# adamgreig/labrador-ldpc

Measured on AMD Instinct MI355X. Metric: decoded codewords/sec @25 min-sum iters, TM8192, Eb/N0=2dB; 1/2/4/8 GPU, higher is better.
Workload: dtype f32; 1 GPU; TM8192 f32 LLRs, 4194304 frames on 1 GPU = BASELINE config 4 whole, resident in HBM, max_iters 25 with early termination, AWGN Eb/N0 2.0 dB, 256 random codewords; code=TM8192, total_frames=4194304, frames_per_gpu=4194304, max_iters=25, parallelism=1 contiguous shard(s) of one batch, one process per GPU, no collective, kernel_variant=0, library_build=d4d007dc8df32436

## Files before the change

labrador_ldpc_amd/csrc/decode_ms_ops.hpp:

```cpp
#pragma once

#include <hip/hip_runtime.h>
#include <cfloat>
#include <cstdint>
#include <type_traits>

#include "decode_ms_util.hpp"

namespace ldpc {

template <class T> struct Ops;

template <> struct Ops<float> {
    using R = float;
    using E = float;
    LDPC_DEV static R zero() { return 0.0f; }
    LDPC_DEV static R maxval() { return FLT_MAX; }
    LDPC_DEV static R load(float x) { return __builtin_fminf(x + 0.0f, __builtin_inff()); }
    LDPC_DEV static R canon_late(R x) { return __builtin_fminf(x + 0.0f, __builtin_inff()); }
    LDPC_DEV static R keep_raw(float x) { return x; }
    LDPC_DEV static R load_nonan(float x) { return x + 0.0f; }
    LDPC_DEV static float store(R x) { return x; }
    LDPC_DEV static R from_lds(float x) { return x; }
    LDPC_DEV static int bits(R x) { return __float_as_int(x); }
    static constexpr bool SIGN_WORD_IS_BIT31_ONLY = true;
    LDPC_DEV static int sign_word(R x) { return __float_as_int(x) & (int)0x80000000; }
    LDPC_DEV static R add(R a, R b) { return a + b; }
    LDPC_DEV static R sub(R a, R b) { return a - b; }
    LDPC_DEV static R sub_nv(R a, R b) { return a - b; }
    LDPC_DEV static R mag(R x) { return __builtin_fabsf(x); }
    template <bool AX, bool AY>
    LDPC_DEV static R min2(R x, R y)
    {
        R d;
        if constexpr (AX && AY) asm("v_min_f32_e64 %0, |%1|, |%2|" : "=v"(d) : "v"(x), "v"(y));
        else if constexpr (AX) asm("v_min_f32_e64 %0, |%1|, %2" : "=v"(d) : "v"(x), "v"(y));
        else if constexpr (AY) asm("v_min_f32_e64 %0, %1, |%2|" : "=v"(d) : "v"(x), "v"(y));
        else asm("v_min_f32_e32 %0, %1, %2" : "=v"(d) : "v"(x), "v"(y));
        return d;
    }
    template <bool AX>
    LDPC_DEV static R min2_cap(R x)
    {
        R d;
        const float cap = FLT_MAX;
        if constexpr (AX) asm("v_min_f32_e64 %0, |%1|, %2" : "=v"(d) : "v"(x), "s"(cap));
        else asm("v_min_f32_e32 %0, %2, %1" : "=v"(d) : "v"(x), "s"(cap));
        return d;
    }
    template <bool AX, bool AY>
    LDPC_DEV static R min3_cap(R x, R y)
    {
        R d;
        const float cap = FLT_MAX;
        if constexpr (AX && AY) asm("v_min3_f32 %0, |%1|, |%2|, %3" : "=v"(d) : "v"(x), "v"(y), "s"(cap));
        else if constexpr (!AX && !AY) asm("v_min3_f32 %0, %1, %2, %3" : "=v"(d) : "v"(x), "v"(y), "s"(cap));
        else d = min2_cap<false>(min2<AX, AY>(x, y));
        return d;
    }
    template <bool AX, bool AY, bool AZ>
    LDPC_DEV static R min3(R x, R y, R z)
    {
        R d;
        if constexpr (AX && AY && AZ) asm("v_min3_f32 %0, |%1|, |%2|, |%3|" : "=v"(d) : "v"(x), "v"(y), "v"(z));
        else if constexpr (AX && AY) asm("v_min3_f32 %0, |%1|, |%2|, %3" : "=v"(d) : "v"(x), "v"(y), "v"(z));
        else if constexpr (!AX && !AY && !AZ) asm("v_min3_f32 %0, %1, %2, %3" : "=v"(d) : "v"(x), "v"(y), "v"(z));
        else d = min2<false, AZ>(min2<AX, AY>(x, y), z);
        return d;
    }
    LDPC_DEV static R with_sign(R m, int s)
    {
        return __int_as_float((__float_as_int(m) & 0x7FFFFFFF) | (s & (int)0x80000000));
    }
    LDPC_DEV static R select_zero(bool z, R x) { return z ? 0.0f : x; }
    LDPC_DEV static R keep_unless_negative(R p, R x)
    {
        R r;
        asm("v_subrev_co_u32_e32 %0, vcc, %2, %1\n\ts_nop 1\n\tv_cndmask_b32_e32 %0, 0, %3, vcc"
            : "=&v"(r) : "v"(p), "s"(0x80000001u), "v"(x) : "vcc");
        return r;
    }
    LDPC_DEV static bool drop(R nv, R old)
    {
        const int t = __builtin_amdgcn_bitop3_b32(__float_as_int(old), __float_as_int(nv), (int)0x80000000, 0x78);
        return __int_as_float(t) < 0.0f;
    }
    template <int FORM>
    LDPC_DEV static R clamp_to_side(R nv, R old, float big)
    {
        static_assert(FORM == 2 || FORM == 3, "clamp forms of the self-correction: 2, 3 (6: integer messages only, IntOps)");
        R x, r;
        if constexpr (FORM == 2) {
            asm("v_fma_f32 %0, %1, %2, %3" : "=v"(x) : "s"(big), "v"(old), "v"(nv));
        } else {
            asm("v_mul_legacy_f32_e64 %0, %1, %2" : "=v"(x) : "v"(old), "s"(__builtin_inff()));
            x = x + nv;
        }
        asm("v_med3_f32 %0, %1, 0, %2" : "=v"(r) : "v"(nv), "v"(x));
        return r;
    }
    template <int FORM>
    LDPC_DEV static R self_correct(R nv, R old)
    {
        if constexpr (FORM == 1) {
            const int t = __builtin_amdgcn_bitop3_b32(__float_as_int(old), __float_as_int(nv), (int)0x80000000, 0x78);
            return keep_unless_negative(__int_as_float(t), nv);
        } else {
            return select_zero(drop(nv, old), nv);
        }
    }
    template <bool BOUNDED, int FORM = 0>
    LDPC_DEV static R self_correct_b(R nv, R old)
    {
        if constexpr (BOUNDED && FORM >= 2) {
            return clamp_to_side<FORM>(nv, old, 0x1p126f);
        } else if constexpr (BOUNDED) {
            float p;
            asm("v_mul_f32_e32 %0, %1, %2" : "=v"(p) : "v"(nv), "v"(old));
            if constexpr (FORM == 1) return keep_unless_negative(p, nv);
            else return select_zero(p < 0.0f, nv);
        } else {
            return self_correct<(FORM == 1 ? 1 : 0)>(nv, old);
        }
    }
    LDPC_DEV static R apply_sign(R m, int s_all, int s_own)
    {
        return __int_as_float(__builtin_amdgcn_bitop3_b32(__float_as_int(m), s_all, s_own, 0x96));
    }
};

template <> struct Ops<double> {
    using R = double;
    using E = double;
    LDPC_DEV static R zero() { return 0.0; }
    LDPC_DEV static R maxval() { return DBL_MAX; }
    LDPC_DEV static R load(double x) { return __builtin_fmin(x + 0.0, __builtin_inf()); }
    LDPC_DEV static R canon_late(R x) { return __builtin_fmin(x + 0.0, __builtin_inf()); }
    LDPC_DEV static R keep_raw(double x) { return x; }
    LDPC_DEV static R load_nonan(double x) { return x + 0.0; }
    LDPC_DEV static double store(R x) { return x; }
    LDPC_DEV static R from_lds(double x) { return x; }
    LDPC_DEV static int bits(R x) { return __double2hiint(x); }
    static constexpr bool SIGN_WORD_IS_BIT31_ONLY = true;
    LDPC_DEV static int sign_word(R x) { return __double2hiint(x) & (int)0x80000000; }
    LDPC_DEV static R add(R a, R b) { return a + b; }
    LDPC_DEV static R sub(R a, R b) { return a - b; }
    LDPC_DEV static R sub_nv(R a, R b) { return a - b; }
    LDPC_DEV static R mag(R x) { return __builtin_fabs(x); }
    template <bool AX, bool AY>
    LDPC_DEV static R min2(R x, R y)
    {
        const R a = AX ? __builtin_fabs(x) : x, b = AY ? __builtin_fabs(y) : y;
        return __builtin_fmin(a, b);
    }
    template <bool AX> LDPC_DEV static R min2_cap(R x) { return min2<AX, false>(x, DBL_MAX); }
    template <bool AX, bool AY> LDPC_DEV static R min3_cap(R x, R y) { return min2<false, false>(min2<AX, AY>(x, y), DBL_MAX); }
    template <bool AX, bool AY, bool AZ>
    LDPC_DEV static R min3(R x, R y, R z) { return min2<false, AZ>(min2<AX, AY>(x, y), z); }
    template <int FORM>
    LDPC_DEV static R self_correct(R nv, R old)
    {
        return (old != 0.0 && (nv < 0.0) != (old < 0.0)) ? 0.0 : nv;
    }
    template <bool BOUNDED, int FORM = 0> LDPC_DEV static R self_correct_b(R nv, R old) { return self_correct<0>(nv, old); }
    LDPC_DEV static R apply_sign(R m, int s_all, int s_own)
    {
        return __hiloint2double(__double2hiint(m) ^ s_all ^ s_own, __double2loint(m));
    }
};

template <class I, int LO, int HI> struct IntOps : Ops<float> {
    LDPC_DEV static R maxval() { return (float)HI; }
    LDPC_DEV static R load(I x) { return (float)(int)x; }
    LDPC_DEV static R canon_late(R x) { return x; }
    LDPC_DEV static R keep_raw(I x) { return (float)(int)x; }
    LDPC_DEV static R load_nonan(I x) { return (float)(int)x; }
    LDPC_DEV static R clamp(R x) { return __builtin_amdgcn_fmed3f(x, (float)LO, (float)HI); }
    LDPC_DEV static R add(R a, R b) { return clamp(a + b); }
    LDPC_DEV static R sub(R a, R b) { return clamp(a - b); }
    LDPC_DEV static R sub_nv(R a, R b) { return a - b; }
    LDPC_DEV static R mag(R x) { return __builtin_fminf(__builtin_fabsf(x), (float)HI); }
    LDPC_DEV static bool drop(R nv, R old)
    {
        float p;
        asm("v_mul_f32_e32 %0, %1, %2" : "=v"(p) : "v"(nv), "v"(old));
        return p < 0.0f;
    }
    template <int FORM>
    LDPC_DEV static R self_correct(R nv, R old)
    {
        if constexpr (FORM == 6) {
            float sel, r;
            asm("v_fma_f32 %0, %1, %2, 1.0 clamp" : "=v"(sel) : "v"(nv), "v"(old));
            asm("v_fma_f32 %0, %1, %2, 0" : "=v"(r) : "v"(nv), "v"(sel));
            return r;
        } else if constexpr (FORM >= 2) {
            return Ops<float>::clamp_to_side<FORM>(nv, old, 0x1p20f);
        } else if constexpr (FORM == 1) {
            float p;
            asm("v_mul_f32_e32 %0, %1, %2" : "=v"(p) : "v"(nv), "v"(old));
            return Ops<float>::keep_unless_negative(p, nv);
        } else {
            return Ops<float>::select_zero(drop(nv, old), nv);
        }
    }
    template <bool BOUNDED, int FORM = 0> LDPC_DEV static R self_correct_b(R nv, R old) { return self_correct<FORM>(nv, old); }
    template <bool AX>
    LDPC_DEV static R min2_cap(R x)
    {
        R d;
        const float cap = (float)HI;
        if constexpr (AX) asm("v_min_f32_e64 %0, |%1|, %2" : "=v"(d) : "v"(x), "s"(cap));
        else asm("v_min_f32_e32 %0, %2, %1" : "=v"(d) : "v"(x), "s"(cap));
        return d;
    }
    template <bool AX, bool AY>
    LDPC_DEV static R min3_cap(R x, R y)
    {
        R d;
        const float cap = (float)HI;
        if constexpr (AX && AY) asm("v_min3_f32 %0, |%1|, |%2|, %3" : "=v"(d) : "v"(x), "v"(y), "s"(cap));
        else if constexpr (!AX && !AY) asm("v_min3_f32 %0, %1, %2, %3" : "=v"(d) : "v"(x), "v"(y), "s"(cap));
        else d = min2_cap<false>(Ops<float>::min2<AX, AY>(x, y));
        return d;
    }
};
template <> struct Ops<int8_t>  : IntOps<int8_t, -128, 127> {};
template <> struct Ops<int16_t> : IntOps<int16_t, -32768, 32767> {};

template <> struct Ops<int32_t> {
    using R = int;
    using E = float;
    LDPC_DEV static R zero() { return 0; }
    LDPC_DEV static R maxval() { return 0x7FFFFFFF; }
    LDPC_DEV static R load(int32_t x) { return x; }
    LDPC_DEV static R canon_late(R x) { return x; }
    LDPC_DEV static R keep_raw(int32_t x) { return x; }
    LDPC_DEV static R load_nonan(int32_t x) { return x; }
    LDPC_DEV static float store(R x) { return __int_as_float(x); }
    LDPC_DEV static R from_lds(float x) { return __float_as_int(x); }
    LDPC_DEV static int bits(R x) { return x; }
    static constexpr bool SIGN_WORD_IS_BIT31_ONLY = true;
    LDPC_DEV static int sign_word(R x) { return x & (int)0x80000000; }
    LDPC_DEV static R add(R a, R b) { R d; asm("v_add_i32 %0, %1, %2 clamp" : "=v"(d) : "v"(a), "v"(b)); return d; }
    LDPC_DEV static R sub(R a, R b) { R d; asm("v_sub_i32 %0, %1, %2 clamp" : "=v"(d) : "v"(a), "v"(b)); return d; }
    LDPC_DEV static R sub_nv(R a, R b) { return sub(a, b); }
    LDPC_DEV static R mag(R x) { const R s = x >> 31; return (R)((unsigned)(x ^ s) - (unsigned)s); }
    LDPC_DEV static R umin(R a, R b) { return (unsigned)b < (unsigned)a ? b : a; }
    template <bool AX, bool AY>
    LDPC_DEV static R min2(R x, R y)
    {
        const R a = AX ? mag(x) : x, b = AY ? mag(y) : y;
        return umin(a, b);
    }
    template <bool AX> LDPC_DEV static R min2_cap(R x) { return umin(AX ? mag(x) : x, maxval()); }
    template <bool AX, bool AY> LDPC_DEV static R min3_cap(R x, R y) { return umin(min2<AX, AY>(x, y), maxval()); }
    template <bool AX, bool AY, bool AZ>
    LDPC_DEV static R min3(R x, R y, R z) { return min2<false, AZ>(min2<AX, AY>(x, y), z); }
    template <int FORM>
    LDPC_DEV static R self_correct(R nv, R old)
    {
        const int negold = (int)(0u - (unsigned)old);
        const int drop = __builtin_amdgcn_bitop3_b32(nv, old, negold, 0x2C) >> 31;
        return __builtin_amdgcn_bitop3_b32(nv, drop, drop, 0x30);
    }
    template <bool BOUNDED, int FORM = 0> LDPC_DEV static R self_correct_b(R nv, R old) { return self_correct<0>(nv, old); }
    LDPC_DEV static R apply_sign(R m, int s_all, int s_own)
    {
        const int k = (s_all ^ s_own) >> 31;
        return (m ^ k) - k;
    }
};

template <class O, int D, bool ABS, bool CAP = true>
LDPC_DEV void exclusive_min(const typename O::R (&a)[D], typename O::R (&e)[D])
{
    using R = typename O::R;
    const R MX = O::maxval();
    if constexpr (D == 1) {
        e[0] = MX;
    } else if constexpr (D == 2) {
        if constexpr (CAP) {
            e[0] = O::template min2_cap<ABS>(a[1]);
            e[1] = O::template min2_cap<ABS>(a[0]);
        } else {
            e[0] = ABS ? O::mag(a[1]) : a[1];
            e[1] = ABS ? O::mag(a[0]) : a[0];
        }
    } else if constexpr (D == 3) {
        e[0] = O::template min3_cap<ABS, ABS>(a[1], a[2]);
        e[1] = O::template min3_cap<ABS, ABS>(a[0], a[2]);
        e[2] = O::template min3_cap<ABS, ABS>(a[0], a[1]);
    } else {
        constexpr int G = (D + 2) / 3;
        R t[G], x[G];
        static_for<0, G>([&](auto g_) LDPC_INLINE {
            constexpr int g = decltype(g_)::value, n = (3 * g + 3 <= D) ? 3 : D - 3 * g;
            if constexpr (n == 3) t[g] = O::template min3<ABS, ABS, ABS>(a[3 * g], a[3 * g + 1], a[3 * g + 2]);
            else if constexpr (n == 2) t[g] = O::template min2<ABS, ABS>(a[3 * g], a[3 * g + 1]);
            else t[g] = ABS ? O::mag(a[3 * g]) : a[3 * g];
        });
        exclusive_min<O, G, false, CAP>(t, x);
        static_for<0, G>([&](auto g_) LDPC_INLINE {
            constexpr int g = decltype(g_)::value, n = (3 * g + 3 <= D) ? 3 : D - 3 * g;
            if constexpr (n == 3) {
                e[3 * g]     = O::template min3<ABS, ABS, false>(a[3 * g + 1], a[3 * g + 2], x[g]);
                e[3 * g + 1] = O::template min3<ABS, ABS, false>(a[3 * g],     a[3 * g + 2], x[g]);
                e[3 * g + 2] = O::template min3<ABS, ABS, false>(a[3 * g],     a[3 * g + 1], x[g]);
            } else if constexpr (n == 2) {
                e[3 * g]     = O::template min2<ABS, false>(a[3 * g + 1], x[g]);
                e[3 * g + 1] = O::template min2<ABS, false>(a[3 * g],     x[g]);
            } else {
                e[3 * g] = x[g];
            }
        });
    }
}

template <class T, class R>
LDPC_DEV T soft_value(R x)
{
    if constexpr (std::is_same_v<T, int8_t> || std::is_same_v<T, int16_t>) return (T)(int)x;
    else return (T)x;
}

}
```

labrador_ldpc_amd/csrc/decode_ms_pair.hpp:

```cpp
#pragma once

#include "decode_ms_kernel.hpp"


namespace ldpc {


typedef float ldpc_f2 __attribute__((ext_vector_type(2)));

template <int CODE, class T>
struct PairGeometry {
    static constexpr int M = CODES[CODE].m;
    static constexpr int NT = M / 2;
    static constexpr int NX = count_exchanged(*CODES[CODE].proto);
    static constexpr int NXC = count_exch_cols(*CODES[CODE].proto);
    static constexpr int OUT_LEN = CODES[CODE].output_len();
    static constexpr int LDS_BYTES = ((NX + NXC) * M * 4 + 16 + 15) / 16 * 16;
    static_assert(M % 512 == 0 && NT <= 1024, "pair ownership needs M/8 >= 64 lanes per quarter and <= 1024 threads");
};

constexpr int pair_local_rank(const Prototype &p, int S, int B)
{
    int nloc = 0, r = 0;
    for (int b = 0; b < p.n_blocks; ++b)
        if (blk_local(p.blk[b])) { if (b < B) ++r; ++nloc; }
    return S * nloc + r;
}

constexpr bool all_exchanged_are_pi(const Prototype &p)
{
    for (int b = 0; b < p.n_blocks; ++b)
        if (!blk_local(p.blk[b]) && p.blk[b].kind != BLK_P) return false;
    return true;
}

template <class T, bool SOFT, bool CORRECTED>
constexpr int pair_hoist_addresses()
{
    if (LDPC_PAIR_HOIST >= 0) return LDPC_PAIR_HOIST;
    return (std::is_same_v<T, float> && !SOFT && !CORRECTED) ? LDPC_PAIR_HOIST_F32 : 0;
}

constexpr int pair_var_read_block(const Prototype &p, int k)
{
    for (int c = 0; c < p.n_cols; ++c)
        for (int b = 0; b < p.n_blocks; ++b)
            if (p.blk[b].col == c && exch_slot(p, b) >= 0 && k-- == 0) return b;
    return -1;
}
constexpr int pair_var_read_rank(const Prototype &p, int B)
{
    for (int k = 0; k < p.n_blocks; ++k)
        if (pair_var_read_block(p, k) == B) return k;
    return -1;
}

template <int HOIST, int NX>
constexpr int pair_early_u()
{
    if (HOIST == 0 || LDPC_PAIR_PEEL_FIRST == 0) return 0;
    if (LDPC_PAIR_EARLY_U >= 0) return LDPC_PAIR_EARLY_U < NX ? LDPC_PAIR_EARLY_U : NX;
    return LDPC_PAIR_EARLY_U_F32 < NX ? LDPC_PAIR_EARLY_U_F32 : NX;
}

template <int CODE, class T, int JW, int FORM, bool SOFT = false, bool CORRECTED = false>
LDPC_DEV void decode_ms_pair_body(const T *__restrict__ llrs, uint8_t *__restrict__ output,
                                  uint32_t *__restrict__ iters_out, uint8_t *__restrict__ success_out,
                                  uint32_t batch, uint32_t maxiters, float nocap_limit, uint32_t *claim, char *lds,
                                  T *__restrict__ app = nullptr, float corr_scale = 1.0f, float corr_offset = 0.0f)
{
    static_assert(!CORRECTED || std::is_same_v<T, float>, "the correction step is built for f32 messages");
    using GEO = PairGeometry<CODE, T>;
    using O = Ops<T>;
    using R = typename O::R;
    static_assert(sizeof(R) == 4 && sizeof(typename O::E) == 4, "pair kernel: 4-byte message types");
    constexpr Prototype P = *CODES[CODE].proto;
    static_assert(all_exchanged_are_pi(P), "pair kernel: exchanged blocks must be pi_k");
    constexpr int M = GEO::M, NT = GEO::NT, NB = P.n_blocks, NROWS = P.n_rows, NCOLS = P.n_cols;
    constexpr int N = CODES[CODE].n, NTX = N / M, NX = GEO::NX, NXC = GEO::NXC;
    constexpr int Q = M / 4, IPT = 2;
    constexpr int BLK_BYTES = M * 4, FLAG_OFF = (NX + NXC) * BLK_BYTES;
    constexpr bool ODD_B64 = LDPC_PAIR_ODD_B64 >= 0 ? LDPC_PAIR_ODD_B64 != 0 : true;
    constexpr int LOCAL_IN_VAR = LDPC_PAIR_LOCAL_IN_VAR >= 0 ? LDPC_PAIR_LOCAL_IN_VAR : (std::is_same_v<T, float> ? 10 : 8);
    constexpr int HOIST = pair_hoist_addresses<T, SOFT, CORRECTED>();
    constexpr int EARLY = pair_early_u<HOIST, NX>();
    static_assert(EARLY >= 0 && EARLY <= 15, "lgkmcnt counts to 15");
    constexpr bool PRIO_WAVES = true;
    (void)PRIO_WAVES;

    const int t = (int)(threadIdx.x & (M / 8 - 1)) + JW * (M / 8);
    __builtin_assume(t >= 0 && t < NT);
    const uint32_t n_groups = batch;
    uint32_t cw = blockIdx.x;
    bool live = cw < batch;
    (void)live;

    auto lds1 = [&](int off) LDPC_INLINE -> float & { return *reinterpret_cast<float *>(lds + off); };
    auto lds2 = [&](int off) LDPC_INLINE -> ldpc_f2 & { return *reinterpret_cast<ldpc_f2 *>(lds + off); };
    auto flag_at = [&](uint32_t which) LDPC_INLINE -> int & { return *reinterpret_cast<int *>(lds + FLAG_OFF + 4 * (which & 1)); };
    auto cap_flag = [&]() LDPC_INLINE -> int & { return *reinterpret_cast<int *>(lds + FLAG_OFF + 8); };
    constexpr bool NOCAP_POSSIBLE = LDPC_PAIR_NOCAP && std::is_same_v<T, float>;

    auto even_c = [](int B) constexpr { return (phi_of(P.blk[B].val, JW, M) & 1) == 0; };
    auto wire = [&](auto B_, auto S_, int tb8) LDPC_INLINE -> int {
        constexpr int B = decltype(B_)::value, S = decltype(S_)::value;
        constexpr int K = P.blk[B].val;
        constexpr int base = (((theta_of(K) + JW) & 3) * Q) * 4 + lds_bias(P, B, BLK_BYTES);
        return ((tb8 + (phi_of(K, JW, M) + S) * 4) & (Q * 4 - 1)) | base;
    };

    R u[IPT][NB], v[IPT][NB], va[IPT][NCOLS], llr[IPT][NTX];
    int fnext = 0;
    (void)fnext;
    ldpc_f2 upre[EARLY > 0 ? EARLY : 1];
    (void)upre;
    T lraw[IPT][NTX];

    auto fetch_llrs = [&](uint32_t c) LDPC_INLINE {
        unsigned tu = (unsigned)t;
        asm volatile("" : "+v"(tu));
        const uint32_t cc = c < batch ? c : batch - 1;
        static_for<0, NTX>([&](auto C_) LDPC_INLINE {
            constexpr int C = decltype(C_)::value;
            const T *src = (llrs + (size_t)cc * N) + (unsigned)(C * M);
            lraw[0][C] = src[2 * tu];
            lraw[1][C] = src[2 * tu + 1];
        });
    };

    auto forget_llrs = [&]() LDPC_INLINE {
        static_for<0, IPT>([&](auto S_) LDPC_INLINE {
            static_for<0, NTX>([&](auto C_) LDPC_INLINE {
                if constexpr (sizeof(T) == 4) { T &x = lraw[decltype(S_)::value][decltype(C_)::value]; asm volatile("" : "=v"(x)); }
            });
        });
    };
    (void)forget_llrs;
    constexpr int VB_HI = 0x10000;
    int had[IPT][NB], vb[2];
    (void)had; (void)vb;
    auto hoist_addresses = [&]() LDPC_INLINE {
        int tq = t;
        asm volatile("" : "+v"(tq));
        const int tb8 = tq * 8;
        vb[0] = tb8;
        asm volatile("" : "+v"(vb[0]));
        if constexpr (FLAG_OFF > VB_HI) {
            vb[1] = tb8 + VB_HI;
            asm volatile("" : "+v"(vb[1]));
        }
        static_for<0, NB>([&](auto B_) LDPC_INLINE {
            constexpr int B = decltype(B_)::value;
            if constexpr (exch_slot(P, B) >= 0) {
                constexpr int lo = lds_bias(P, B, BLK_BYTES);
                static_assert(lds_xu_off(P, exch_slot(P, B), BLK_BYTES) - lo + 4 < 0x10000 && lds_xva_off(P, col_slot(P, P.blk[B].col), BLK_BYTES) - lo + 4 < 0x10000);
                if constexpr (even_c(B)) {
                    had[0][B] = wire(B_, IC<0>{}, tb8);
                } else if constexpr (ODD_B64) {
                    had[0][B] = wire(B_, IC<-1>{}, tb8);
                    had[1][B] = wire(B_, IC<1>{}, tb8);
                    asm volatile("" : "+v"(had[1][B]));
                } else {
                    had[0][B] = wire(B_, IC<0>{}, tb8);
                    had[1][B] = wire(B_, IC<1>{}, tb8);
                    asm volatile("" : "+v"(had[1][B]));
                }
                asm volatile("" : "+v"(had[0][B]));
            }
        });
    };
    auto own = [&](auto OFF_) LDPC_INLINE -> int {
        constexpr int off = decltype(OFF_)::value;
        if constexpr (off < VB_HI) return vb[0] + off;
        else return vb[1] + (off - VB_HI);
    };
    (void)own;

    auto begin_codeword = [&]() LDPC_INLINE {
        if constexpr (HOIST == 1) hoist_addresses();
        int tq = t;
        asm volatile("" : "+v"(tq));
        const int tb8 = tq * 8;
        static_for<0, IPT>([&](auto S_) LDPC_INLINE {
            constexpr int S = decltype(S_)::value;
            static_for<0, NB>([&](auto B_) LDPC_INLINE {
                constexpr int B = decltype(B_)::value;
                u[S][B] = O::zero();
                v[S][B] = O::zero();
            });
            static_for<0, NCOLS>([&](auto C_) LDPC_INLINE { va[S][decltype(C_)::value] = O::zero(); });
            static_for<0, NTX>([&](auto C_) LDPC_INLINE { llr[S][decltype(C_)::value] = O::load(lraw[S][decltype(C_)::value]); });
        });
        if constexpr (!LDPC_PAIR_PEEL_FIRST)
        static_for<0, NX>([&](auto X_) LDPC_INLINE {
            lds2(lds_xu_off(P, decltype(X_)::value, BLK_BYTES) + tb8) = ldpc_f2{0.0f, 0.0f};
        });
        if (t < 2) flag_at(t) = 0;
        if constexpr (NOCAP_POSSIBLE) {
            bool big = false;
            static_for<0, IPT>([&](auto S_) LDPC_INLINE {
                static_for<0, NTX>([&](auto C_) LDPC_INLINE {
                    const R a = O::mag(llr[decltype(S_)::value][decltype(C_)::value]);
                    big |= !(a <= nocap_limit) || (a != 0.0f && a < 0x1p-20f);
                });
            });
            if (__ballot(big) != 0 && (t & 63) == 0) cap_flag() = 1;
        }
    };

    auto edge_update = [&](auto S_, auto B_, R x, auto BND_) LDPC_INLINE {
        constexpr int S = decltype(S_)::value, B = decltype(B_)::value;
        const R nv = O::sub_nv(x, u[S][B]);
        constexpr bool BND = decltype(BND_)::value != 0;
        constexpr int F = (FORM >= 2 && (BND || sizeof(T) <= 2)) ? FORM : (LDPC_PAIR_SELFCORR_CARRY != 0 ? 1 : 0);
        v[S][B] = O::template self_correct_b<BND, F>(nv, v[S][B]);
    };

    auto variable_phase = [&](auto BND_, auto FIRST_) LDPC_INLINE {
        constexpr bool FIRST = decltype(FIRST_)::value != 0;
        constexpr bool PRE = EARLY > 0 && !FIRST;
        (void)PRE;
        int tq = t;
        if constexpr (HOIST == 0) asm volatile("" : "+v"(tq));
        const int tb8 = tq * 8;
        (void)tb8;
        LDPC_SETPRIO(LDPC_PRIO_VAR);
        static_for<0, NCOLS>([&](auto C_) LDPC_INLINE {
            constexpr int C = decltype(C_)::value;
            if constexpr (C == NCOLS / 2) LDPC_SETPRIO(0);
            R acc0 = O::zero(), acc1 = O::zero();
            if constexpr (C < NTX) { acc0 = llr[0][C]; acc1 = llr[1][C]; }
            if constexpr (!FIRST)
            static_for<0, NB>([&](auto B_) LDPC_INLINE {
                constexpr int B = decltype(B_)::value;
                if constexpr (P.blk[B].col == C) {
                    constexpr int slot = exch_slot(P, B);
                    if constexpr (slot >= 0) {
                        ldpc_f2 up;
                        constexpr int rank = pair_var_read_rank(P, B);
                        if constexpr (PRE && rank < EARLY) {
                            ldpc_f2 &x = upre[rank];
                            asm volatile("s_waitcnt lgkmcnt(%1)" : "+v"(x) : "n"(EARLY - 1 - rank));
                            up = x;
                        }
                        else if constexpr (HOIST != 0) up = lds2(own(IC<lds_xu_off(P, slot, BLK_BYTES)>{}));
                        else up = lds2(lds_xu_off(P, slot, BLK_BYTES) + tb8);
                        acc0 = O::add(acc0, O::from_lds(up.x));
                        acc1 = O::add(acc1, O::from_lds(up.y));
                    } else {
                        acc0 = O::add(acc0, u[0][B]);
                        acc1 = O::add(acc1, u[1][B]);
                    }
                }
            });
            va[0][C] = acc0;
            va[1][C] = acc1;
            constexpr int cs = col_slot(P, C);
            if constexpr (cs >= 0) {
                if constexpr (HOIST != 0) lds2(own(IC<lds_xva_off(P, cs, BLK_BYTES)>{})) = ldpc_f2{O::store(acc0), O::store(acc1)};
                else lds2(lds_xva_off(P, cs, BLK_BYTES) + tb8) = ldpc_f2{O::store(acc0), O::store(acc1)};
            }
        });
        static_for<0, IPT>([&](auto S_) LDPC_INLINE {
            static_for<0, NB>([&](auto B_) LDPC_INLINE {
                constexpr int S = decltype(S_)::value, B = decltype(B_)::value;
                if constexpr (exch_slot(P, B) < 0 && pair_local_rank(P, S, B) < LOCAL_IN_VAR) {
                    if constexpr (FIRST) v[S][B] = va[S][P.blk[B].col];
                    else edge_update(S_, B_, va[S][P.blk[B].col], BND_);
                }
            });
        });
    };

    auto check_phase = [&](uint32_t it, auto CAP_, auto FIRST_) LDPC_INLINE {
        constexpr bool CAP = decltype(CAP_)::value != 0;
        constexpr bool FIRST = decltype(FIRST_)::value != 0;
        constexpr int BND = (!CAP && NOCAP_POSSIBLE) ? 1 : 0;
        int par_any = 0;
        int tq = t;
        if constexpr (HOIST == 0) asm volatile("" : "+v"(tq));
        const int tb8 = tq * 8;
        (void)tb8;
        LDPC_SETPRIO(3);
        R xs[IPT][NB];
        int ad[IPT][NB];
        auto request_marginals = [&]() LDPC_INLINE {
        static_for<0, NB>([&](auto B_) LDPC_INLINE {
            constexpr int B = decltype(B_)::value;
            constexpr int slot = exch_slot(P, B);
            if constexpr (slot >= 0) {
                constexpr int cs = col_slot(P, P.blk[B].col);
                constexpr int off = lds_xva_off(P, cs, BLK_BYTES) - lds_bias(P, B, BLK_BYTES);
                if constexpr (HOIST != 0) {
                    ad[0][B] = had[0][B];
                    if constexpr (!even_c(B)) ad[1][B] = had[1][B];
                }
                if constexpr (even_c(B)) {
                    if constexpr (HOIST == 0) ad[0][B] = wire(B_, IC<0>{}, tb8);
                    const ldpc_f2 xp = lds2(off + ad[0][B]);
                    xs[0][B] = O::from_lds(xp.x);
                    xs[1][B] = O::from_lds(xp.y);
                } else if constexpr (ODD_B64) {
                    if constexpr (HOIST == 0) {
                        ad[0][B] = wire(B_, IC<-1>{}, tb8);
                        ad[1][B] = wire(B_, IC<1>{}, tb8);
                    }
                    const ldpc_f2 lo = lds2(off + ad[0][B]), hi = lds2(off + ad[1][B]);
                    xs[0][B] = O::from_lds(lo.y);
                    xs[1][B] = O::from_lds(hi.x);
                } else {
                    if constexpr (HOIST == 0) {
                        ad[0][B] = wire(B_, IC<0>{}, tb8);
                        ad[1][B] = wire(B_, IC<1>{}, tb8);
                    }
                    xs[0][B] = O::from_lds(lds1(off + ad[0][B]));
                    xs[1][B] = O::from_lds(lds1(off + ad[1][B]));
                }
            }
        });
        };
        auto local_edges = [&]() LDPC_INLINE {
        static_for<0, IPT>([&](auto S_) LDPC_INLINE {
            static_for<0, NB>([&](auto B_) LDPC_INLINE {
                constexpr int S = decltype(S_)::value, B = decltype(B_)::value;
                if constexpr (exch_slot(P, B) < 0 && pair_local_rank(P, S, B) >= LOCAL_IN_VAR) {
                    if constexpr (FIRST) v[S][B] = va[S][P.blk[B].col];
                    else edge_update(S_, B_, va[S][P.blk[B].col], IC<BND>{});
                }
            });
        });
        };
        request_marginals();
        __builtin_amdgcn_sched_barrier(0);
        local_edges();
        __builtin_amdgcn_sched_barrier(0);
        static_for<0, IPT>([&](auto S_) LDPC_INLINE {
            static_for<0, NB>([&](auto B_) LDPC_INLINE {
                constexpr int S = decltype(S_)::value, B = decltype(B_)::value;
                if constexpr (exch_slot(P, B) >= 0) {
                    if constexpr (FIRST) v[S][B] = xs[S][B];
                    else edge_update(S_, B_, xs[S][B], IC<BND>{});
                }
            });
        });
        static_for<0, NROWS>([&](auto R_) LDPC_INLINE {
            constexpr int Rw = decltype(R_)::value;
            constexpr int D = row_degree(P, Rw);
            static_for<0, IPT>([&](auto S_) LDPC_INLINE {
                constexpr int S = decltype(S_)::value;
                {
                    constexpr int prio_rows[6] = LDPC_PRIO_ROWS_PAIR;
                    constexpr int step = Rw * IPT + S, nsteps = IPT * NROWS;
                    constexpr int k = step - (nsteps - 6);
                    constexpr int now = k >= 0 ? prio_rows[k] : 3, before = (step > 0 && k >= 1) ? prio_rows[k - 1] : 3;
                    if constexpr (now != before) LDPC_SETPRIO(now);
                }
                R a[D], e[D];
                int sr[D], xw[D];
                static_for<0, D>([&](auto J_) LDPC_INLINE {
                    constexpr int J = decltype(J_)::value;
                    constexpr int B = row_block(P, Rw, J);
                    a[J] = v[S][B];
                    sr[J] = O::sign_word(v[S][B]);
                    if constexpr (exch_slot(P, B) >= 0) xw[J] = O::bits(xs[S][B]);
                    else xw[J] = O::bits(va[S][P.blk[B].col]);
                });
                const int sgn = xor_reduce<D>(sr), par = xor_reduce<D>(xw);
                exclusive_min<O, D, true, CAP>(a, e);
                if constexpr (CORRECTED)
                    static_for<0, D>([&](auto J_) LDPC_INLINE {
                        constexpr int J = decltype(J_)::value;
                        e[J] = __builtin_fmaxf(__fsub_rn(__fmul_rn(corr_scale, e[J]), corr_offset), 0.0f);
                    });
                static_for<0, D>([&](auto J_) LDPC_INLINE {
                    constexpr int J = decltype(J_)::value;
                    constexpr int B = row_block(P, Rw, J);
                    u[S][B] = O::apply_sign(e[J], sgn, sr[J]);
                    constexpr int slot = exch_slot(P, B);
                    if constexpr (slot >= 0) {
                        constexpr int off = lds_xu_off(P, slot, BLK_BYTES) - lds_bias(P, B, BLK_BYTES);
                        if constexpr (!even_c(B)) lds1(off + ad[S][B] + (ODD_B64 && S == 0 ? 4 : 0)) = O::store(u[S][B]);
                        else if constexpr (S == 1) lds2(off + ad[0][B]) = ldpc_f2{O::store(u[0][B]), O::store(u[1][B])};
                    }
                });
                par_any |= par;
            });
        });
        if constexpr (EARLY > 0 && !FIRST) { if (par_any < 0) *reinterpret_cast<int *>(lds + fnext) = 1; }
        else if (par_any < 0) flag_at(it) = 1;
    };

    if (t == 0) cap_flag() = 0;
    if constexpr (HOIST == 2) hoist_addresses();
    LDPC_SYNC();
    constexpr bool FETCH_EARLY = LDPC_PAIR_FETCH_EARLY >= 0 ? LDPC_PAIR_FETCH_EARLY != 0 : sizeof(T) >= 4;
    if (FETCH_EARLY && blockIdx.x < n_groups) fetch_llrs(blockIdx.x);
    const bool dyn = claim != nullptr && maxiters != 0;
    uint32_t ticket = 0;
    int *const next_word = reinterpret_cast<int *>(lds + FLAG_OFF + 12);
    auto collect_claim = [&]() LDPC_INLINE {
        if constexpr (JW == 0) {
            if (dyn && t == 0) {
                *next_word = (int)(gridDim.x + ticket);
                if (ticket == n_groups - 1) __hip_atomic_store(claim, 0u, __ATOMIC_RELAXED, __HIP_MEMORY_SCOPE_AGENT);
            }
        }
    };
    for (uint32_t g = blockIdx.x; g < n_groups;) {
        cw = (uint32_t)__builtin_amdgcn_readfirstlane((int)g);
        if constexpr (JW == 0) {
            if (dyn && t == 0) ticket = __hip_atomic_fetch_add(claim, 1u, __ATOMIC_RELAXED, __HIP_MEMORY_SCOPE_AGENT);
        }
        if constexpr (!FETCH_EARLY) fetch_llrs(cw);
        begin_codeword();
        bool done = false, ok = false;
        uint32_t iters = maxiters;
        auto iterate = [&](auto CAP_) LDPC_INLINE {
            uint32_t it0 = 0;
            if constexpr (LDPC_PAIR_PEEL_FIRST != 0) {
                if (maxiters == 0) { done = true; return; }
                variable_phase(IC<(decltype(CAP_)::value == 0 && NOCAP_POSSIBLE) ? 1 : 0>{}, IC<1>{});
                LDPC_SYNC();
                check_phase(0u, CAP_, IC<1>{});
                collect_claim();
                it0 = 1;
            }
            if constexpr (EARLY > 0) {
                int fsel = FLAG_OFF;
                for (uint32_t it = 1;; ++it) {
                    asm volatile("" : "+s"(it));
                    LDPC_SYNC();
                    int fl, fa;
                    asm volatile("" : "+s"(fsel));
                    asm volatile("v_mov_b32 %0, %2\n\tds_read_b32 %1, %0" : "=&v"(fa), "=v"(fl) : "s"(fsel));
                    static_for<0, EARLY>([&](auto K_) LDPC_INLINE {
                        constexpr int K = decltype(K_)::value;
                        constexpr int off = lds_xu_off(P, exch_slot(P, pair_var_read_block(P, K)), BLK_BYTES);
                        static_assert((off < VB_HI ? off : off - VB_HI) < 0x10000);
                        ldpc_f2 &x = upre[K];
                        const int &base = vb[off < VB_HI ? 0 : 1];
                        asm volatile("ds_read_b64 %0, %1 offset:%2" : "=v"(x) : "v"(base), "n"(off < VB_HI ? off : off - VB_HI));
                    });
                    asm volatile("s_waitcnt lgkmcnt(%1)" : "+v"(fl) : "n"(EARLY));
                    if (__builtin_amdgcn_readfirstlane(fl) == 0) { done = true; ok = true; iters = it - 1; }
                    else if (it == maxiters) { done = true; }
                    if (done) break;
                    variable_phase(IC<(decltype(CAP_)::value == 0 && NOCAP_POSSIBLE) ? 1 : 0>{}, IC<0>{});
                    LDPC_SYNC();
                    if (t == 0) *reinterpret_cast<int *>(lds + fa) = 0;
                    fsel ^= 4;
                    asm volatile("" : "+s"(fsel));
                    fnext = fsel;
                    check_phase(it, CAP_, IC<0>{});
                }
            } else
            for (uint32_t it = it0;; ++it) {
                if (it > 0) LDPC_SYNC();
                if (it > 0 && flag_at(it - 1) == 0) { done = true; ok = true; iters = it - 1; }
                else if (it == maxiters) { done = true; }
                if (done) break;
                variable_phase(IC<(decltype(CAP_)::value == 0 && NOCAP_POSSIBLE) ? 1 : 0>{}, IC<0>{});
                LDPC_SYNC();
                if (it > 0 && t == 0) flag_at(it - 1) = 0;
                check_phase(it, CAP_, IC<0>{});
                if constexpr (LDPC_PAIR_PEEL_FIRST == 0) { if (it == 0) collect_claim(); }
            }
        };
        LDPC_SYNC();
        if constexpr (NOCAP_POSSIBLE) {
            if (__builtin_amdgcn_readfirstlane(cap_flag()) != 0) iterate(IC<1>{});
            else iterate(IC<0>{});
        } else {
            iterate(IC<1>{});
        }
        if constexpr (EARLY > 0) {
            asm volatile("s_waitcnt lgkmcnt(0)");
            __builtin_amdgcn_sched_barrier(0);
        }
        const uint32_t g_next = dyn ? (uint32_t)__builtin_amdgcn_readfirstlane(*next_word) : g + gridDim.x;
        if (FETCH_EARLY && g_next < n_groups) fetch_llrs(g_next);
        else if constexpr (HOIST != 0 && FETCH_EARLY && sizeof(T) == 4) forget_llrs();
        static_for<0, NCOLS>([&](auto C_) LDPC_INLINE {
            constexpr int C = decltype(C_)::value;
            const unsigned long long ev = __ballot(O::bits(va[0][C]) < 0), od = __ballot(O::bits(va[1][C]) < 0);
            unsigned long long w[2];
            static_for<0, 2>([&](auto H_) LDPC_INLINE {
                constexpr int H = decltype(H_)::value;
                unsigned long long re, ro;
                const unsigned e32 = (unsigned)(ev >> (32 * H)), o32 = (unsigned)(od >> (32 * H));
                asm("s_bitreplicate_b64_b32 %0, %1" : "=s"(re) : "s"(e32));
                asm("s_bitreplicate_b64_b32 %0, %1" : "=s"(ro) : "s"(o32));
                const unsigned long long il = (re & 0x5555555555555555ull) | (ro & 0xAAAAAAAAAAAAAAAAull);
                const unsigned lo = __builtin_bswap32(__builtin_bitreverse32((unsigned)il));
                const unsigned hi = __builtin_bswap32(__builtin_bitreverse32((unsigned)(il >> 32)));
                w[H] = (unsigned long long)lo | ((unsigned long long)hi << 32);
            });
            if constexpr (SOFT) {
                struct alignas(2 * sizeof(T)) Pair { T e, o; };
                unsigned tu = (unsigned)t;
                asm volatile("" : "+v"(tu));
                Pair *const dst_app = reinterpret_cast<Pair *>(app + (size_t)cw * (NCOLS * M) + C * M + 2 * tu);
                Pair pr{soft_value<T>(va[0][C]), soft_value<T>(va[1][C])};
                *dst_app = pr;
                if constexpr (std::is_floating_point_v<T> && C < NTX) {
                    if (__ballot(va[0][C] == __builtin_inff() || va[1][C] == __builtin_inff()) != 0) {
                        const T *src = (llrs + (size_t)cw * N) + (unsigned)(C * M) + 2 * tu;
                        const T x0 = src[0], x1 = src[1];
                        pr.e = x0 != x0 ? x0 : pr.e;
                        pr.o = x1 != x1 ? x1 : pr.o;
                        *dst_app = pr;
                    }
                }
            }
            if ((t & 63) == 0) {
                unsigned long long *dst = reinterpret_cast<unsigned long long *>((output + (size_t)cw * GEO::OUT_LEN) + (C * M + 2 * t) / 8);
                dst[0] = w[0];
                dst[1] = w[1];
            }
        });
        if (t == 0) { iters_out[cw] = iters; success_out[cw] = ok ? 1 : 0; cap_flag() = 0; }
        LDPC_SYNC();
        g = g_next;
    }
}

template <class T>
constexpr int pair_form_default()
{
    if (LDPC_PAIR_SELFCORR_MED3 >= 0) return LDPC_PAIR_SELFCORR_MED3;
    if (sizeof(T) <= 2) return 6;
    return (sizeof(T) > 4 || std::is_same_v<T, int32_t>) ? 0 : 2;
}

template <int CODE, class T, int FORM = pair_form_default<T>()>
__global__ void __launch_bounds__((PairGeometry<CODE, T>::NT))
decode_ms_pair_kernel(const T *__restrict__ llrs, uint8_t *__restrict__ output, uint32_t *__restrict__ iters_out,
                      uint8_t *__restrict__ success_out, uint32_t batch, uint32_t maxiters, float nocap_limit, uint32_t *claim)
{
    using GEO = PairGeometry<CODE, T>;
    __shared__ __attribute__((aligned(16))) char lds[GEO::LDS_BYTES];
    const int jw = __builtin_amdgcn_readfirstlane((int)threadIdx.x) / (GEO::M / 8);
    if (jw == 0) decode_ms_pair_body<CODE, T, 0, FORM>(llrs, output, iters_out, success_out, batch, maxiters, nocap_limit, claim, lds);
    else if (jw == 1) decode_ms_pair_body<CODE, T, 1, FORM>(llrs, output, iters_out, success_out, batch, maxiters, nocap_limit, claim, lds);
    else if (jw == 2) decode_ms_pair_body<CODE, T, 2, FORM>(llrs, output, iters_out, success_out, batch, maxiters, nocap_limit, claim, lds);
    else decode_ms_pair_body<CODE, T, 3, FORM>(llrs, output, iters_out, success_out, batch, maxiters, nocap_limit, claim, lds);
}

template <int CODE, class T, int FORM = pair_form_default<T>()>
__global__ void __launch_bounds__((PairGeometry<CODE, T>::NT))
soft_decode_ms_pair_kernel(const T *__restrict__ llrs, T *__restrict__ app, uint8_t *__restrict__ output, uint32_t *__restrict__ iters_out,
                           uint8_t *__restrict__ success_out, uint32_t batch, uint32_t maxiters, float nocap_limit, uint32_t *claim)
{
    using GEO = PairGeometry<CODE, T>;
    __shared__ __attribute__((aligned(16))) char lds[GEO::LDS_BYTES];
    const int jw = __builtin_amdgcn_readfirstlane((int)threadIdx.x) / (GEO::M / 8);
    if (jw == 0) decode_ms_pair_body<CODE, T, 0, FORM, true>(llrs, output, iters_out, success_out, batch, maxiters, nocap_limit, claim, lds, app);
    else if (jw == 1) decode_ms_pair_body<CODE, T, 1, FORM, true>(llrs, output, iters_out, success_out, batch, maxiters, nocap_limit, claim, lds, app);
    else if (jw == 2) decode_ms_pair_body<CODE, T, 2, FORM, true>(llrs, output, iters_out, success_out, batch, maxiters, nocap_limit, claim, lds, app);
    else decode_ms_pair_body<CODE, T, 3, FORM, true>(llrs, output, iters_out, success_out, batch, maxiters, nocap_limit, claim, lds, app);
}

}
```

labrador_ldpc_amd/csrc/decode_ms_tuning.hpp:

```cpp
#pragma once

#ifndef LDPC_TUNING_OVERRIDES_ALLOWED
#if defined(LDPC_QUARTER_SPECIALISE) || defined(LDPC_NOCAP) || defined(LDPC_LOCAL_IN_VAR) || defined(LDPC_PRIO) || defined(LDPC_PRIO_ROWS) || \
    defined(LDPC_PRIO_ROWS_LEAN) || defined(LDPC_PRIO_VAR) || defined(LDPC_TM2048_WAVES) || defined(LDPC_PAIR_LOCAL_IN_VAR) || defined(LDPC_PAIR_NOCAP) || \
    defined(LDPC_PAIR_ODD_B64) || defined(LDPC_PRIO_ROWS_PAIR) || defined(LDPC_SELFCORR_CARRY) || defined(LDPC_WAVE_VERDICT) || defined(LDPC_WG_VERDICT) || \
    defined(LDPC_PEEL_FIRST) || defined(LDPC_PAIR_PEEL_FIRST) || defined(LDPC_PAIR_FETCH_EARLY) || defined(LDPC_PAIR_SELFCORR_CARRY) || \
    defined(LDPC_SELFCORR_MED3) || defined(LDPC_PAIR_SELFCORR_MED3) || defined(LDPC_LEAN_CH) || \
    defined(LDPC_PAIR_HOIST) || defined(LDPC_PAIR_HOIST_F32) || defined(LDPC_PAIR_EARLY_U) || defined(LDPC_PAIR_EARLY_U_F32)
#error "the LDPC_* tuning switches are fixed in a library build (kernel experiments: tools/kbench/)"
#endif
#endif

#ifndef LDPC_QUARTER_SPECIALISE
#define LDPC_QUARTER_SPECIALISE 2
#endif
#ifndef LDPC_SELFCORR_CARRY
#define LDPC_SELFCORR_CARRY -1
#endif
#ifndef LDPC_SELFCORR_MED3
#define LDPC_SELFCORR_MED3 -1
#endif
#ifndef LDPC_PAIR_SELFCORR_MED3
#define LDPC_PAIR_SELFCORR_MED3 -1
#endif
#ifndef LDPC_PAIR_FETCH_EARLY
#define LDPC_PAIR_FETCH_EARLY -1
#endif
#ifndef LDPC_PAIR_PEEL_FIRST
#define LDPC_PAIR_PEEL_FIRST 1
#endif
#ifndef LDPC_PAIR_SELFCORR_CARRY
#define LDPC_PAIR_SELFCORR_CARRY 0
#endif
#ifndef LDPC_WAVE_VERDICT
#define LDPC_WAVE_VERDICT 1
#endif
#ifndef LDPC_PEEL_FIRST
#define LDPC_PEEL_FIRST -1
#endif
#ifndef LDPC_WG_VERDICT
#define LDPC_WG_VERDICT -1
#endif
#ifndef LDPC_NOCAP
#define LDPC_NOCAP 1
#endif
#ifndef LDPC_LOCAL_IN_VAR
#define LDPC_LOCAL_IN_VAR -1
#endif
#ifndef LDPC_PRIO
#define LDPC_PRIO 2
#endif
#ifndef LDPC_PRIO_ROWS
#define LDPC_PRIO_ROWS {2, 2, 1, 1, 1, 0}
#endif
#ifndef LDPC_LEAN_CH
#define LDPC_LEAN_CH 6
#endif
#ifndef LDPC_PRIO_ROWS_LEAN
#define LDPC_PRIO_ROWS_LEAN {3, 3, 3, 2, 1, 0}
#endif
#ifndef LDPC_PRIO_VAR
#define LDPC_PRIO_VAR 2
#endif
#ifndef LDPC_TM2048_WAVES
#define LDPC_TM2048_WAVES 6
#endif

#ifndef LDPC_PAIR_LOCAL_IN_VAR
#define LDPC_PAIR_LOCAL_IN_VAR -1
#endif
#ifndef LDPC_PAIR_NOCAP
#define LDPC_PAIR_NOCAP 1
#endif
#ifndef LDPC_PAIR_ODD_B64
#define LDPC_PAIR_ODD_B64 -1
#endif
#ifndef LDPC_PAIR_HOIST
#define LDPC_PAIR_HOIST -1
#endif
#ifndef LDPC_PAIR_HOIST_F32
#define LDPC_PAIR_HOIST_F32 2
#endif
#ifndef LDPC_PAIR_EARLY_U
#define LDPC_PAIR_EARLY_U -1
#endif
#ifndef LDPC_PAIR_EARLY_U_F32
#define LDPC_PAIR_EARLY_U_F32 8
#endif

#ifndef LDPC_PRIO_ROWS_PAIR
#define LDPC_PRIO_ROWS_PAIR {3, 3, 2, 2, 1, 0}
#endif
```

Baseline: 9.457 million codewords/s.

## Defer finishing local-edge check messages into the LDS read wait window

For the f32 pair kernel with early u reads, the check phase now computes only the partial group minima and signs for the first few local (non-exchanged) edges. The final min and sign application for those edges runs after the exchanged-message LDS reads are issued and before the lgkmcnt wait. The aim is to fill the LDS latency gap with useful ALU work and shorten the check phase's critical path. In exchange the kernel holds extra registers (dx, dsg), which may raise register pressure, and LOCAL_IN_VAR gets a new default when deferral is on.

```diff
diff --git a/labrador_ldpc_amd/csrc/decode_ms_ops.hpp b/labrador_ldpc_amd/csrc/decode_ms_ops.hpp
--- a/labrador_ldpc_amd/csrc/decode_ms_ops.hpp
+++ b/labrador_ldpc_amd/csrc/decode_ms_ops.hpp
@@ -317,6 +317,38 @@
     }
 }
 
+template <int D>
+constexpr bool exclusive_min_has_part() { return D >= 4; }
+
+template <class O, int D, bool ABS, bool CAP, int GRP>
+LDPC_DEV typename O::R exclusive_min_part(const typename O::R (&a)[D])
+{
+    static_assert(D >= 4, "rows of degree <= 3 are finished from their elements alone");
+    using R = typename O::R;
+    constexpr int G = (D + 2) / 3;
+    R t[G], x[G];
+    static_for<0, G>([&](auto g_) LDPC_INLINE {
+        constexpr int g = decltype(g_)::value, n = (3 * g + 3 <= D) ? 3 : D - 3 * g;
+        if constexpr (n == 3) t[g] = O::template min3<ABS, ABS, ABS>(a[3 * g], a[3 * g + 1], a[3 * g + 2]);
+        else if constexpr (n == 2) t[g] = O::template min2<ABS, ABS>(a[3 * g], a[3 * g + 1]);
+        else t[g] = ABS ? O::mag(a[3 * g]) : a[3 * g];
+    });
+    exclusive_min<O, G, false, CAP>(t, x);
+    return x[GRP];
+}
+
+template <class O, int D, bool ABS, int J>
+LDPC_DEV typename O::R exclusive_min_finish(const typename O::R (&a)[D], typename O::R xg)
+{
+    static_assert(D >= 3, "rows of degree 1 and 2 have nothing to finish");
+    constexpr int g = J / 3, n = (3 * g + 3 <= D) ? 3 : D - 3 * g;
+    constexpr int o0 = 3 * g + (J % 3 == 0 ? 1 : 0), o1 = 3 * g + (J % 3 == 2 ? 1 : 2);
+    if constexpr (D == 3) return O::template min3_cap<ABS, ABS>(a[o0], a[o1]);
+    else if constexpr (n == 3) return O::template min3<ABS, ABS, false>(a[o0], a[o1], xg);
+    else if constexpr (n == 2) return O::template min2<ABS, false>(a[3 * g + 1 - J % 3], xg);
+    else return xg;
+}
+
 template <class T, class R>
 LDPC_DEV T soft_value(R x)
 {
diff --git a/labrador_ldpc_amd/csrc/decode_ms_pair.hpp b/labrador_ldpc_amd/csrc/decode_ms_pair.hpp
--- a/labrador_ldpc_amd/csrc/decode_ms_pair.hpp
+++ b/labrador_ldpc_amd/csrc/decode_ms_pair.hpp
@@ -61,6 +61,42 @@
     if (HOIST == 0 || LDPC_PAIR_PEEL_FIRST == 0) return 0;
     if (LDPC_PAIR_EARLY_U >= 0) return LDPC_PAIR_EARLY_U < NX ? LDPC_PAIR_EARLY_U : NX;
     return LDPC_PAIR_EARLY_U_F32 < NX ? LDPC_PAIR_EARLY_U_F32 : NX;
+}
+
+constexpr int pair_defer_rank(const Prototype &p, int S, int B)
+{
+    int r = 0;
+    for (int b = 0; b < p.n_blocks; ++b)
+        if (blk_local(p.blk[b])) {
+            if (p.blk[b].row < p.blk[B].row) r += 2;
+            else if (p.blk[b].row == p.blk[B].row) r += (S == 1 ? 1 : 0) + (b < B ? 1 : 0);
+        }
+    return r;
+}
+constexpr bool pair_deferred(const Prototype &p, int S, int B, int defer)
+{
+    return blk_local(p.blk[B]) && pair_defer_rank(p, S, B) < defer;
+}
+constexpr bool pair_defer_first_of_group(const Prototype &p, int S, int row, int j, int defer)
+{
+    for (int k = j / 3 * 3; k < j; ++k)
+        if (pair_deferred(p, S, row_block(p, row, k), defer)) return false;
+    return true;
+}
+constexpr int count_local(const Prototype &p)
+{
+    int c = 0;
+    for (int b = 0; b < p.n_blocks; ++b) c += blk_local(p.blk[b]) ? 1 : 0;
+    return c;
+}
+
+template <int CODE, int JW, int EARLY>
+constexpr int pair_defer_local()
+{
+    constexpr int nloc = 2 * count_local(*CODES[CODE].proto);
+    if (EARLY == 0) return 0;
+    if (LDPC_PAIR_DEFER_LOCAL >= 0) return LDPC_PAIR_DEFER_LOCAL < nloc ? LDPC_PAIR_DEFER_LOCAL : nloc;
+    return LDPC_PAIR_DEFER_LOCAL_F32 < nloc ? LDPC_PAIR_DEFER_LOCAL_F32 : nloc;
 }
 
 template <int CODE, class T, int JW, int FORM, bool SOFT = false, bool CORRECTED = false>
@@ -81,10 +117,13 @@
     constexpr int Q = M / 4, IPT = 2;
     constexpr int BLK_BYTES = M * 4, FLAG_OFF = (NX + NXC) * BLK_BYTES;
     constexpr bool ODD_B64 = LDPC_PAIR_ODD_B64 >= 0 ? LDPC_PAIR_ODD_B64 != 0 : true;
-    constexpr int LOCAL_IN_VAR = LDPC_PAIR_LOCAL_IN_VAR >= 0 ? LDPC_PAIR_LOCAL_IN_VAR : (std::is_same_v<T, float> ? 10 : 8);
     constexpr int HOIST = pair_hoist_addresses<T, SOFT, CORRECTED>();
     constexpr int EARLY = pair_early_u<HOIST, NX>();
     static_assert(EARLY >= 0 && EARLY <= 15, "lgkmcnt counts to 15");
+    constexpr int DEFER = pair_defer_local<CODE, JW, EARLY>();
+    static_assert(DEFER == 0 || (EARLY > 0 && !SOFT && !CORRECTED), "deferred local edges: the instantiations with early u reads");
+    constexpr int LOCAL_IN_VAR = LDPC_PAIR_LOCAL_IN_VAR >= 0 ? LDPC_PAIR_LOCAL_IN_VAR
+                                 : DEFER > 0 ? LDPC_PAIR_LOCAL_IN_VAR_DEFER : (std::is_same_v<T, float> ? 10 : 8);
     constexpr bool PRIO_WAVES = true;
     (void)PRIO_WAVES;
 
@@ -114,6 +153,9 @@
     (void)fnext;
     ldpc_f2 upre[EARLY > 0 ? EARLY : 1];
     (void)upre;
+    int dsg[IPT][NROWS];
+    R dx[IPT][NROWS][(NB + 2) / 3];
+    (void)dsg; (void)dx;
     T lraw[IPT][NTX];
 
     auto fetch_llrs = [&](uint32_t c) LDPC_INLINE {
@@ -215,6 +257,30 @@
         constexpr int F = (FORM >= 2 && (BND || sizeof(T) <= 2)) ? FORM : (LDPC_PAIR_SELFCORR_CARRY != 0 ? 1 : 0);
         v[S][B] = O::template self_correct_b<BND, F>(nv, v[S][B]);
     };
+
+    auto finish_deferred = [&]() LDPC_INLINE {
+        static_for<0, NROWS>([&](auto R_) LDPC_INLINE {
+            constexpr int Rw = decltype(R_)::value;
+            constexpr int D = row_degree(P, Rw);
+            static_for<0, IPT>([&](auto S_) LDPC_INLINE {
+                constexpr int S = decltype(S_)::value;
+                R a[D];
+                static_for<0, D>([&](auto J_) LDPC_INLINE { a[decltype(J_)::value] = v[S][row_block(P, Rw, decltype(J_)::value)]; });
+                static_for<0, D>([&](auto J_) LDPC_INLINE {
+                    constexpr int J = decltype(J_)::value;
+                    constexpr int B = row_block(P, Rw, J);
+                    if constexpr (pair_deferred(P, S, B, DEFER)) {
+                        R xg = O::zero();
+                        if constexpr (exclusive_min_has_part<D>()) xg = dx[S][Rw][J / 3];
+                        const R e = exclusive_min_finish<O, D, true, J>(a, xg);
+                        u[S][B] = O::apply_sign(e, dsg[S][Rw], O::sign_word(v[S][B]));
+                        asm volatile("" : "+v"(u[S][B]));
+                    }
+                });
+            });
+        });
+    };
+    (void)finish_deferred;
 
     auto variable_phase = [&](auto BND_, auto FIRST_) LDPC_INLINE {
         constexpr bool FIRST = decltype(FIRST_)::value != 0;
@@ -372,9 +438,24 @@
                         constexpr int J = decltype(J_)::value;
                         e[J] = __builtin_fmaxf(__fsub_rn(__fmul_rn(corr_scale, e[J]), corr_offset), 0.0f);
                     });
+                if constexpr (DEFER > 0) {
+                    bool any = false;
+                    static_for<0, D>([&](auto J_) LDPC_INLINE {
+                        constexpr int J = decltype(J_)::value;
+                        if constexpr (pair_deferred(P, S, row_block(P, Rw, J), DEFER)) {
+                            any = true;
+                            constexpr bool first = pair_defer_first_of_group(P, S, Rw, J, DEFER);
+                            if constexpr (exclusive_min_has_part<D>() && first) {
+                                dx[S][Rw][J / 3] = exclusive_min_part<O, D, true, CAP, J / 3>(a);
+                            }
+                        }
+                    });
+                    if (any) dsg[S][Rw] = sgn;
+                }
                 static_for<0, D>([&](auto J_) LDPC_INLINE {
                     constexpr int J = decltype(J_)::value;
                     constexpr int B = row_block(P, Rw, J);
+                    if constexpr (pair_deferred(P, S, B, DEFER)) return;
                     u[S][B] = O::apply_sign(e[J], sgn, sr[J]);
                     constexpr int slot = exch_slot(P, B);
                     if constexpr (slot >= 0) {
@@ -441,6 +522,11 @@
                         const int &base = vb[off < VB_HI ? 0 : 1];
                         asm volatile("ds_read_b64 %0, %1 offset:%2" : "=v"(x) : "v"(base), "n"(off < VB_HI ? off : off - VB_HI));
                     });
+                    if constexpr (DEFER > 0) {
+                        __builtin_amdgcn_sched_barrier(0);
+                        finish_deferred();
+                        __builtin_amdgcn_sched_barrier(0);
+                    }
                     asm volatile("s_waitcnt lgkmcnt(%1)" : "+v"(fl) : "n"(EARLY));
                     if (__builtin_amdgcn_readfirstlane(fl) == 0) { done = true; ok = true; iters = it - 1; }
                     else if (it == maxiters) { done = true; }
diff --git a/labrador_ldpc_amd/csrc/decode_ms_tuning.hpp b/labrador_ldpc_amd/csrc/decode_ms_tuning.hpp
--- a/labrador_ldpc_amd/csrc/decode_ms_tuning.hpp
+++ b/labrador_ldpc_amd/csrc/decode_ms_tuning.hpp
@@ -6,7 +6,8 @@
     defined(LDPC_PAIR_ODD_B64) || defined(LDPC_PRIO_ROWS_PAIR) || defined(LDPC_SELFCORR_CARRY) || defined(LDPC_WAVE_VERDICT) || defined(LDPC_WG_VERDICT) || \
     defined(LDPC_PEEL_FIRST) || defined(LDPC_PAIR_PEEL_FIRST) || defined(LDPC_PAIR_FETCH_EARLY) || defined(LDPC_PAIR_SELFCORR_CARRY) || \
     defined(LDPC_SELFCORR_MED3) || defined(LDPC_PAIR_SELFCORR_MED3) || defined(LDPC_LEAN_CH) || \
-    defined(LDPC_PAIR_HOIST) || defined(LDPC_PAIR_HOIST_F32) || defined(LDPC_PAIR_EARLY_U) || defined(LDPC_PAIR_EARLY_U_F32)
+    defined(LDPC_PAIR_HOIST) || defined(LDPC_PAIR_HOIST_F32) || defined(LDPC_PAIR_EARLY_U) || defined(LDPC_PAIR_EARLY_U_F32) || \
+    defined(LDPC_PAIR_DEFER_LOCAL) || defined(LDPC_PAIR_DEFER_LOCAL_F32) || defined(LDPC_PAIR_LOCAL_IN_VAR_DEFER)
 #error "the LDPC_* tuning switches are fixed in a library build (kernel experiments: tools/kbench/)"
 #endif
 #endif
@@ -87,6 +88,15 @@
 #ifndef LDPC_PAIR_EARLY_U_F32
 #define LDPC_PAIR_EARLY_U_F32 8
 #endif
+#ifndef LDPC_PAIR_DEFER_LOCAL
+#define LDPC_PAIR_DEFER_LOCAL -1
+#endif
+#ifndef LDPC_PAIR_DEFER_LOCAL_F32
+#define LDPC_PAIR_DEFER_LOCAL_F32 6
+#endif
+#ifndef LDPC_PAIR_LOCAL_IN_VAR_DEFER
+#define LDPC_PAIR_LOCAL_IN_VAR_DEFER 12
+#endif
 
 #ifndef LDPC_PRIO_ROWS_PAIR
 #define LDPC_PRIO_ROWS_PAIR {3, 3, 2, 2, 1, 0}
```

New measurement: 9.683 million codewords/s, median of 6. +2.4%, better.
